# Tai-Wang/Depth-from-Motion

Hardware: AMD Instinct MI355X
Metric: cost-volumes/sec (higher is better)
Workload: dtype bf16; 1 GPU; nstar: plane-sweep cost-volume build B=8/GPU x (2C=512, D=112, 94x311), feats 256x94x311 bf16, fsf=4 csf=1; global_batch=8, parallelism=dp1, kernel=sweep_tile_kernel<LDS>, launch=lanes256_ppl8_planes2_chunk1_pipelined_cut64, autotuned=True, volume_layout=(B,2C,D,H,W) contiguous (the reference layout)

## Files before the change

### depth-from-motion_amd/csrc/plane_sweep.hip

```cpp
#include "plane_sweep_common.h"

#include <stdlib.h>
#include <string.h>

#include <algorithm>
#include <map>
#include <mutex>
#include <vector>

using namespace dfm;

namespace {

thread_local int g_last_kernel = 0;
#ifdef DFM_DEBUG_HOOKS
unsigned long long *g_trace = nullptr;
#endif

struct Launch {
    int kernel;
    int lanes;
    int lds_kib;
    int bpg;
    int planes;
    int band_chunk;
    int ppl;
    int align;
    int pair;
    int unpack;
    int pipe;
};

struct TuneKey {
    int v[9];
    bool operator<(const TuneKey &o) const { return memcmp(v, o.v, sizeof(v)) < 0; }
};
std::mutex g_tune_mu;
std::map<TuneKey, dfm_sweep_opts> g_tuned;

constexpr int PACK_PPL = 1;
__global__ void sweep_reset_kernel(int *flags, int n_flags, int *b, int *c)
{
    for (int i = threadIdx.x; i < n_flags; i += blockDim.x) flags[i] = 0;
    if (threadIdx.x == 0) { *b = 0; *c = 0; }
}

template <typename T>
__global__ __launch_bounds__(256) void pack_blocked_kernel(const T *__restrict__ src0,
                                                           const T *__restrict__ src1,
                                                           uint4 *__restrict__ dst0,
                                                           uint4 *__restrict__ dst1, int batch,
                                                           int C, int HW, int nblk, int *__restrict__ flags,
                                                           int W)
{
    constexpr int CB = elem<T>::CB;
    const int pix0 = blockIdx.x * (256 * PACK_PPL) + threadIdx.x;
    const int blk = blockIdx.y;
    const bool second = (int)blockIdx.z >= batch;
    const int b = second ? blockIdx.z - batch : blockIdx.z;
    const T *__restrict__ src = (second ? src1 : src0) + ((size_t)b * C + (size_t)blk * CB) * HW;
    uint4 *__restrict__ dst = (second ? dst1 : dst0) + ((size_t)b * nblk + blk) * HW;
    T v[PACK_PPL][CB];
#pragma unroll
    for (int i = 0; i < PACK_PPL; ++i) {
        const int pix = pix0 + i * 256;
#pragma unroll
        for (int j = 0; j < CB; ++j)
            v[i][j] = (blk * CB + j < C && pix < HW) ? src[(size_t)j * HW + pix] : T(0);
    }
#pragma unroll
    for (int i = 0; i < PACK_PPL; ++i) {
        const int pix = pix0 + i * 256;
        if (pix < HW) {
            uint4 q;
            memcpy(&q, v[i], 16);
            dst[pix] = q;
            if constexpr (sizeof(T) == 2) {
                bool odd_value = false;
                const uint32_t w4[4] = {q.x, q.y, q.z, q.w};
#pragma unroll
                for (int k = 0; k < 4; ++k)
#pragma unroll
                    for (int hbit = 0; hbit < 32; hbit += 16) {
                        const uint32_t e = (w4[k] >> hbit) & 0xffffu, ex = e & 0x7f80u;
                        odd_value |= ex == 0x7f80u || (ex == 0u && e != 0u);
                    }
                if (flags && odd_value) {
                    int *f = flags + (size_t)blockIdx.z * (HW / W) + pix / W;
                    if (__builtin_nontemporal_load(f) == 0) atomicOr(f, 1);
                }
            }
        }
    }
}

template <int CB>
__device__ __forceinline__ void blend(const Tap &t, const uint4 &qnw, const uint4 &qne,
                                      const uint4 &qsw, const uint4 &qse, float (&r)[CB])
{
    float a[CB], b[CB], c[CB], d[CB];
    unpack16(qnw, a);
    unpack16(qne, b);
    unpack16(qsw, c);
    unpack16(qse, d);
    const bool k0 = t.ok & 1u, k1 = t.ok & 2u, k2 = t.ok & 4u, k3 = t.ok & 8u;
#pragma unroll
    for (int j = 0; j < CB; ++j) {
        const float vnw = k0 ? a[j] : 0.0f;
        const float vne = k1 ? b[j] : 0.0f;
        const float vsw = k2 ? c[j] : 0.0f;
        const float vse = k3 ? d[j] : 0.0f;
        float acc = vnw * t.nw;
        acc = __builtin_fmaf(vne, t.ne, acc);
        acc = __builtin_fmaf(vsw, t.sw, acc);
        acc = __builtin_fmaf(vse, t.se, acc);
        r[j] = acc;
    }
}

template <int CB>
__device__ __forceinline__ void blend_nomask(const Tap &t, const uint4 &qnw, const uint4 &qne,
                                             const uint4 &qsw, const uint4 &qse, float (&r)[CB])
{
    float a[CB], b[CB], c[CB], d[CB];
    unpack16(qnw, a);
    unpack16(qne, b);
    unpack16(qsw, c);
    unpack16(qse, d);
#pragma unroll
    for (int j = 0; j < CB; ++j) {
        float acc = a[j] * t.nw;
        acc = __builtin_fmaf(b[j], t.ne, acc);
        acc = __builtin_fmaf(c[j], t.sw, acc);
        acc = __builtin_fmaf(d[j], t.se, acc);
        r[j] = acc;
    }
}

template <typename T>
__global__ __launch_bounds__(256) void sweep_gather_kernel(
    SweepGeom g, const uint4 *__restrict__ cur_blk, const uint4 *__restrict__ prev_blk,
    const float *__restrict__ depths, const float *__restrict__ P, const float *__restrict__ Pinv,
    const float *__restrict__ Tm, T *__restrict__ out)
{
    constexpr int CB = elem<T>::CB;
    const long long n = (long long)blockIdx.x * 256 + threadIdx.x;
    const int b = blockIdx.y;
    if (n >= g.N) return;
    const int hw = g.h_out * g.w_out;
    const int d = (int)(n / hw);
    const int rem = (int)(n - (long long)d * hw);
    const int hi = rem / g.w_out;
    const int wi = rem - hi * g.w_out;

    float cx, cy, px, py;
    sweep_point(g, P + b * 16, Pinv + b * 16, Tm + b * 16, depths[d], hi, wi, cx, cy, px, py,
                nullptr);
    const Tap tc = make_tap(cx, cy, g.h_in, g.w_in);
    const Tap tp = make_tap(px, py, g.h_in, g.w_in);

    const int HW = g.h_in * g.w_in;
    const int c00 = tc.iy * g.w_in + tc.ix, c01 = c00 + tc.dx;
    const int c10 = c00 + tc.dy * g.w_in, c11 = c10 + tc.dx;
    const int p00 = tp.iy * g.w_in + tp.ix, p01 = p00 + tp.dx;
    const int p10 = p00 + tp.dy * g.w_in, p11 = p10 + tp.dx;

    const uint4 *cb = cur_blk + (size_t)b * g.nblk * HW;
    const uint4 *pb = prev_blk + (size_t)b * g.nblk * HW;
    T *ocur = out + ((size_t)b * 2 * g.C) * g.N + n;
    T *oprev = ocur + (size_t)g.C * g.N;

    for (int blk = 0; blk < g.nblk; ++blk) {
        const uint4 qc0 = cb[c00], qc1 = cb[c01], qc2 = cb[c10], qc3 = cb[c11];
        const uint4 qp0 = pb[p00], qp1 = pb[p01], qp2 = pb[p10], qp3 = pb[p11];
// ... 4 lines not shown
#pragma unroll
        for (int j = 0; j < CB; ++j) {
            if (cbase + j < g.C) {
                ocur[(size_t)(cbase + j) * g.N] = elem<T>::store(rc[j]);
                oprev[(size_t)(cbase + j) * g.N] = elem<T>::store(rp[j]);
            }
        }
        cb += HW;
        pb += HW;
    }
}

template <typename T>
__global__ __launch_bounds__(256) void sweep_bwd_kernel(
    SweepGeom g, const T *__restrict__ gout, const float *__restrict__ depths,
    const float *__restrict__ P, const float *__restrict__ Pinv, const float *__restrict__ Tm,
    float *__restrict__ gcur, float *__restrict__ gprev)
{
    const long long n = (long long)blockIdx.x * 256 + threadIdx.x;
    const int b = blockIdx.y;
    if (n >= g.N) return;
    const int hw = g.h_out * g.w_out;
    const int d = (int)(n / hw);
    const int rem = (int)(n - (long long)d * hw);
    const int hi = rem / g.w_out;
    const int wi = rem - hi * g.w_out;
    float cx, cy, px, py;
    sweep_point(g, P + b * 16, Pinv + b * 16, Tm + b * 16, depths[d], hi, wi, cx, cy, px, py,
                nullptr);
    const Tap tc = make_tap(cx, cy, g.h_in, g.w_in);
    const Tap tp = make_tap(px, py, g.h_in, g.w_in);
    const int HW = g.h_in * g.w_in;
    const int c00 = tc.iy * g.w_in + tc.ix, c01 = c00 + tc.dx;
    const int c10 = c00 + tc.dy * g.w_in, c11 = c10 + tc.dx;
    const int p00 = tp.iy * g.w_in + tp.ix, p01 = p00 + tp.dx;
    const int p10 = p00 + tp.dy * g.w_in, p11 = p10 + tp.dx;
    const T *gc = gout + ((size_t)b * 2 * g.C) * g.N + n;
    const T *gp = gc + (size_t)g.C * g.N;
    float *dc = gcur + (size_t)b * g.C * HW;
    float *dp = gprev + (size_t)b * g.C * HW;
    for (int c = 0; c < g.C; ++c) {
        const float go_c = elem<T>::load(gc[(size_t)c * g.N]);
        const float go_p = elem<T>::load(gp[(size_t)c * g.N]);
        if (tc.ok & 1u) atomicAdd(dc + c00, go_c * tc.nw);
        if (tc.ok & 2u) atomicAdd(dc + c01, go_c * tc.ne);
        if (tc.ok & 4u) atomicAdd(dc + c10, go_c * tc.sw);
        if (tc.ok & 8u) atomicAdd(dc + c11, go_c * tc.se);
        if (tp.ok & 1u) atomicAdd(dp + p00, go_p * tp.nw);
        if (tp.ok & 2u) atomicAdd(dp + p01, go_p * tp.ne);
        if (tp.ok & 4u) atomicAdd(dp + p10, go_p * tp.sw);
        if (tp.ok & 8u) atomicAdd(dp + p11, go_p * tp.se);
        dc += HW;
        dp += HW;
    }
}

typedef uint32_t u32x4_t __attribute__((ext_vector_type(4)));

__device__ __forceinline__ void vol_store16(const u32x4_t &v, void *p)
{
    __builtin_nontemporal_store(v, (u32x4_t *)p);
}

__device__ __forceinline__ constexpr int waitcnt_vm(int n)
{
    return (n & 15) | (7 << 4) | (15 << 8) | ((n >> 4) << 14);
}

__device__ __forceinline__ int swz(int q) { return q ^ ((q >> 4) & 7); }

__device__ __forceinline__ uint32_t footprint(float x, float y, int H, int W, int &rN, int &rS,
                                              int &ix, float &fw, float &fn)
{
    const Tap t = make_tap(x, y, H, W);
    ix = (t.ok & 5u) ? t.ix : t.ix - ((t.ok & 10u) ? 1 : 0);
    rN = t.iy;
    rS = t.iy + t.dy;
    const bool fin = (fabsf(x) <= 3.0e38f) && (fabsf(y) <= 3.0e38f);
    fw = fin ? x - floorf(x) : 0.0f;
    fn = fin ? y - floorf(y) : 0.0f;
    return t.ok;
}

struct TileGrid {
    int batch;
    int bands;
    int band_pts;
    int planes;
    int dgroups;
    int blocks_per_group;
    int band_chunk;
    const int *flags;
    int mfma_unpack;
    int pair_stores;
    int align;
    unsigned long long *trace;
    int ablate;
};

constexpr int PIPE_BUF_SLOTS = 2504;
constexpr int PIPE_LDS_BYTES = (8 + 2 * PIPE_BUF_SLOTS) * 16;
template <int N> struct IntC { static constexpr int value = N; };

template <typename T, int NT, bool LDS, int V, bool PIPE = false, bool MXK = false>
__device__ __forceinline__ int tile_body(
    const int bid, const SweepGeom &g, const SweepFast &fast, const TileGrid &tg, int lds_slots,
    const uint4 *__restrict__ cur_blk, const uint4 *__restrict__ prev_blk,
    const float *__restrict__ depths, const float *__restrict__ P,
    const float *__restrict__ Pinv, const float *__restrict__ Tm, T *__restrict__ out,
    int *__restrict__ spill_list, int blk_lo_ovr = -1, int blk_hi_ovr = -1, bool retry_inline = false)
{
    constexpr int CB = elem<T>::CB;
    static_assert(V == 4 || V == 8, "points per lane");
    static_assert(V * sizeof(T) == 16 || V * sizeof(T) == 8, "8- or 16-byte stores");
    static_assert(LDS || !PIPE, "the pipelined body is an LDS-staged body");
    static_assert(!MXK || (LDS && sizeof(T) == 2 && V == 8), "matrix-core unpack: bf16, LDS taps, 8 points per lane");
    constexpr int VW = V * (int)sizeof(T) / 4;
    constexpr int PAD = 8;
    constexpr int SLAB = 8;
    extern __shared__ __attribute__((aligned(16))) uint4 lds[];
    int *bb = (int *)lds;

    const int tid = threadIdx.x;
    const int batch = tg.batch;
    const int b = bid % batch;
    int th = bid / batch;
    const int band_in = th % tg.band_chunk;
    th /= tg.band_chunk;
    const int dgroup = th % tg.dgroups;
    th /= tg.dgroups;
    const int half = th & 1;
    th >>= 1;
    const int nchunks = (tg.bands + tg.band_chunk - 1) / tg.band_chunk;
    const int band = (th % nchunks) * tg.band_chunk + band_in;
    const int group = th / nchunks;
    if (band >= tg.bands) return 0;
    const int blk_lo = blk_lo_ovr >= 0 ? blk_lo_ovr : group * tg.blocks_per_group;
    const int blk_hi = blk_lo_ovr >= 0 ? min(blk_hi_ovr, g.nblk) : min(blk_lo + tg.blocks_per_group, g.nblk);
    const int lanes_per_plane = NT / tg.planes;
    const int d_tile = dgroup * tg.planes + tid / lanes_per_plane;
    const int tid_p = tid % lanes_per_plane;
    const long long hw_ll = (long long)g.h_out * g.w_out;
    const long long a0 = (d_tile * hw_ll) & ~7ll;
    const long long a1 = d_tile >= g.D - 1 ? g.N : (((d_tile + 1) * hw_ll) & ~7ll);
    const long long base = a0 & ~(long long)(tg.align - 1);
    const long long t_end = d_tile < g.D ? min(base + (long long)(band + 1) * tg.band_pts, a1) : 0;
    const long long n0 = base + (long long)band * tg.band_pts + (long long)tid_p * V;
    const bool active = n0 >= a0 && n0 < t_end;
    const int W = g.w_in, H = g.h_in;
    const int HW = H * W;

    if (LDS) {
        if (tid == 0) {
            bb[0] = 0x7fffffff;
            bb[1] = -1;
            lds[SLAB] = make_uint4(0u, 0u, 0u, 0u);
            if constexpr (PIPE) lds[SLAB + PIPE_BUF_SLOTS] = make_uint4(0u, 0u, 0u, 0u);
        }
        __syncthreads();
    }

    int qN[V], qS[V];
    float fw[V], fn[V];
    uint32_t okbits = 0;
    int ymin = 0x7fffffff, ymax = -1;
    if (active) {
        const int hw = g.h_out * g.w_out;
        int d = (int)(n0 / hw);
        int rem = (int)(n0 - (long long)d * hw);
        int hi = rem / g.w_out;
        int wi = rem - hi * g.w_out;
        const float *Pb = P + b * 16, *Pib = Pinv + b * 16, *Tb = Tm + b * 16;
#pragma unroll
        for (int j = 0; j < V; ++j) {
            float sx, sy;
            if (half) sweep_point_map<1>(g, fast, Pb, Pib, Tb, depths[d], hi, wi, sx, sy);
            else sweep_point_map<0>(g, fast, Pb, Pib, Tb, depths[d], hi, wi, sx, sy);
            int rN, rS, ix;
            uint32_t ok = footprint(sx, sy, H, W, rN, rS, ix, fw[j], fn[j]);
            if (LDS && d != d_tile) ok = 0;
            qN[j] = rN * W + ix;
            qS[j] = rS * W + ix;
            okbits |= ok << (4 * j);
            if (ok) { ymin = min(ymin, rN); ymax = max(ymax, rS); }
            if (++wi == g.w_out) { wi = 0; if (++hi == g.h_out) { hi = 0; ++d; } }
            __builtin_amdgcn_sched_barrier(0);
        }
    }
    T *o = out + ((size_t)b * 2 * g.C + (size_t)half * g.C) * g.N + n0;
    const uint32_t full = (V == 8) ? 0xffffffffu : 0xffffu;
    typedef uint32_t u32x2_t __attribute__((ext_vector_type(2)));
    const bool all_in = __all(!active || okbits == full);

    int cnt = 0, nslots = 0;
    int ta[V][4];
    const uint4 *src = (half ? prev_blk : cur_blk) + ((size_t)b * g.nblk + blk_lo) * HW;
    if (LDS) {
#pragma unroll
        for (int s = 32; s > 0; s >>= 1) {
            ymin = min(ymin, __shfl_xor(ymin, s));
            ymax = max(ymax, __shfl_xor(ymax, s));
        }
        if ((tid & 63) == 0) { atomicMin(&bb[0], ymin); atomicMax(&bb[1], ymax); }
        __syncthreads();
        const int y0 = bb[0], y1 = bb[1];
        if (y1 < y0) {
            if (active) {
                for (int c = blk_lo * CB; c < min(blk_hi * CB, g.C); ++c) {
                    if constexpr (VW == 4) {
                        const u32x4_t z = {0u, 0u, 0u, 0u};
                        __builtin_nontemporal_store(z, (u32x4_t *)(o + (size_t)c * g.N));
                    } else {
                        const u32x2_t z = {0u, 0u};
                        __builtin_nontemporal_store(z, (u32x2_t *)(o + (size_t)c * g.N));
                    }
                }
            }
            return 0;
        }
        cnt = (y1 - y0 + 1) * W;
        nslots = (PAD + cnt + 1 + 7) & ~7;
        const bool fits = PIPE ? nslots <= min(PIPE_BUF_SLOTS, (lds_slots - SLAB) / 2)
                               : SLAB + nslots <= lds_slots;
        if (!fits) {
            if (retry_inline) return 1;
            if (tid == 0 && blk_lo_ovr <= 0) spill_list[1 + atomicAdd(&spill_list[0], 1)] = bid;
            return 0;
        }
        if constexpr (MXK) {
            const int nrows = y1 - y0 + 1;
            const int *rf = tg.flags + ((size_t)half * batch + b) * H + y0;
            bool odd_row = false;
            for (int r = tid & 63; r < nrows; r += 64) odd_row |= rf[r] != 0;
            if (__any(odd_row)) {
                if (retry_inline) return 2;
                if (tid == 0 && blk_lo_ovr <= 0) spill_list[1 + atomicAdd(&spill_list[0], 1)] = bid;
                return 0;
            }
        }
        const int off = PAD - y0 * W;
        constexpr int ZERO = SLAB << 4;
#pragma unroll
        for (int j = 0; j < V; ++j) {
            const uint32_t ok = (okbits >> (4 * j)) & 15u;
            const int a = qN[j] + off, c = qS[j] + off;
            ta[j][0] = (ok & 1u) ? (SLAB + swz(a)) << 4 : ZERO;
            ta[j][1] = (ok & 2u) ? (SLAB + swz(a + 1)) << 4 : ZERO;
            ta[j][2] = (ok & 4u) ? (SLAB + swz(c)) << 4 : ZERO;
            ta[j][3] = (ok & 8u) ? (SLAB + swz(c + 1)) << 4 : ZERO;
        }
        src += (size_t)y0 * W;
    } else {
        if (!active) return 0;
#pragma unroll
        for (int j = 0; j < V; ++j) {
            const bool any = (okbits >> (4 * j)) & 15u;
            qN[j] = any ? qN[j] : 0;
            qS[j] = any ? qS[j] : 0;
        }
    }
    const int wave = tid >> 6, lane = tid & 63;
    typedef __bf16 mxs_bf16x4 __attribute__((ext_vector_type(4)));
    mxs_bf16x4 mx_sel;
    if constexpr (MXK) {
        const int i = lane & 3;
        const uint32_t s2[2] = {i == 0 ? 0x3f80u : i == 1 ? 0x3f800000u : 0u,
                                i == 2 ? 0x3f80u : i == 3 ? 0x3f800000u : 0u};
        __builtin_memcpy(&mx_sel, s2, 8);
    }
#ifdef DFM_DEBUG_HOOKS
    unsigned long long *tr = (LDS && tg.trace && (bid % 509) == 0 && tid == 0)
                                 ? tg.trace + (size_t)(bid / 509) * 64 : nullptr;
    int tri = 0;
#endif
#ifndef DFM_DEBUG_HOOKS
#define TRACE_STAMP() do {} while (0)
#define ABLATE(bit) false
#else
#define ABLATE(bit) ((tg.ablate & (bit)) != 0)
#define TRACE_STAMP()                                                                       \
    do {                                                                                    \
        if (tr && tri < 64) {                                                               \
            unsigned long long t_;                                                          \
            asm volatile("s_memtime %0\n\ts_waitcnt lgkmcnt(0)" : "=s"(t_)::"memory");       \
            tr[tri++] = t_;                                                                 \
        }                                                                                   \
    } while (0)
#endif
    TRACE_STAMP();

    auto compute_block = [&](int blk, const uint4 *gsrc, auto bufc, auto mxc, uint32_t (&pk)[CB][VW]) {
        constexpr int BOFF = decltype(bufc)::value * PIPE_BUF_SLOTS * 16;
        constexpr bool MX = decltype(mxc)::value != 0 && MXK;
        static_assert(BOFF < 65536, "ds_read_b128 immediate offset");
        if (ABLATE(4)) {
#pragma unroll
            for (int k = 0; k < CB; ++k)
#pragma unroll
                for (int j = 0; j < VW; ++j) pk[k][j] = (uint32_t)qN[j] + k + blk;
        } else if constexpr (MX) {
            typedef __bf16 mx_bf16x4 __attribute__((ext_vector_type(4)));
            typedef float mx_f32x4 __attribute__((ext_vector_type(4)));
#define DFM_TAP_READ(dst, addr) \
    asm volatile("ds_read_b128 %0, %1 offset:%2" : "=v"(dst) : "v"(addr), "i"(BOFF))
            const mx_f32x4 z4 = {0.0f, 0.0f, 0.0f, 0.0f};
            auto cvt_half = [&](uint32_t lo, uint32_t hi, float *f) {
                mx_bf16x4 bfrag;
                const uint32_t h[2] = {lo, hi};
                __builtin_memcpy(&bfrag, h, 8);
                const mx_f32x4 d4 = __builtin_amdgcn_mfma_f32_4x4x4bf16_1k(mx_sel, bfrag, z4, 0, 0, 0);
                f[0] = d4[0]; f[1] = d4[1]; f[2] = d4[2]; f[3] = d4[3];
            };
            u32x4_t q[2][4];
            float keep[CB];
#pragma unroll
            for (int c4 = 0; c4 < 4; ++c4) DFM_TAP_READ(q[0][c4], ta[0][c4]);
// ... 151 lines not shown
        }
#pragma unroll
        for (int k = 0; k < CB; ++k) {
            if (cbase + k < g.C && (!ABLATE(2) || pk[k][0] == 0x12345u)) {
                if constexpr (VW == 4) {
                    u32x4_t v = {pk[k][0], pk[k][1], pk[k][2], pk[k][3]};
                    vol_store16(v, o + (size_t)(cbase + k) * g.N);
                } else {
                    u32x2_t v = {pk[k][0], pk[k][1]};
                    __builtin_nontemporal_store(v, (u32x2_t *)(o + (size_t)(cbase + k) * g.N));
                }
            }
        }
    };
    auto compute_store = [&](int blk, const uint4 *gsrc, auto bufc, auto mxc) {
        uint32_t pk[CB][VW];
        compute_block(blk, gsrc, bufc, mxc, pk);
        store_block(blk, pk);
    };

    if constexpr (!LDS) {
        for (int blk = blk_lo; blk < blk_hi; ++blk) {
            compute_store(blk, src, IntC<0>{}, IntC<0>{});
            src += HW;
        }
    } else {
        auto stage = [&](int buf_slot0, const uint4 *gsrc) {
            if (ABLATE(1)) return;
            for (int s0 = wave * 64; s0 < nslots; s0 += NT) {
                const int p = swz(s0 + lane) - PAD;
                if (p >= 0 && p < cnt)
                    __builtin_amdgcn_global_load_lds(
                        (const __attribute__((address_space(1))) void *)(gsrc + p),
                        (__attribute__((address_space(3))) void *)(lds + buf_slot0 + s0), 16, 0, 0);
            }
        };
        if constexpr (!PIPE) {
            for (int blk = blk_lo; blk < blk_hi; ++blk) {
                stage(SLAB, src);
                TRACE_STAMP();
                __syncthreads();
                TRACE_STAMP();
                if (active) compute_store(blk, src, IntC<0>{}, IntC<MXK ? 1 : 0>{});
                TRACE_STAMP();
                src += HW;
                __syncthreads();
                TRACE_STAMP();
            }
        } else {
            const bool wave_stores = __any(active) != 0;
            const bool paired = VW == 2 && tg.pair_stores;
            auto wait_rows = [&]() {
                if (wave_stores && !ABLATE(2) && !paired)
                    asm volatile("s_waitcnt vmcnt(%0)\n\ts_barrier" ::"i"(CB) : "memory");
                else if (wave_stores && !ABLATE(2))
                    asm volatile("s_waitcnt vmcnt(%0)\n\ts_barrier" ::"i"(CB / 2) : "memory");
                else
                    asm volatile("s_waitcnt vmcnt(0)\n\ts_barrier" ::: "memory");
            };
            stage(SLAB, src);
            TRACE_STAMP();
            asm volatile("s_waitcnt vmcnt(0) lgkmcnt(0)\n\ts_barrier" ::: "memory");
            for (int blk = blk_lo;;) {
                if (blk + 1 < blk_hi) stage(SLAB + PIPE_BUF_SLOTS, src + HW);
                TRACE_STAMP();
                if (active) compute_store(blk, src, IntC<0>{}, IntC<MXK ? 1 : 0>{});
                TRACE_STAMP();
                src += HW;
                if (++blk >= blk_hi) break;
                wait_rows();
                TRACE_STAMP();
                if (blk + 1 < blk_hi) stage(SLAB, src + HW);
                TRACE_STAMP();
                if (active) compute_store(blk, src, IntC<1>{}, IntC<MXK ? 1 : 0>{});
                TRACE_STAMP();
                src += HW;
                if (++blk >= blk_hi) break;
                wait_rows();
                TRACE_STAMP();
            }
        }
    }
#undef DFM_TAP_READ
    return 0;
}

#ifndef DFM_TILE_WAVES
#define DFM_TILE_WAVES 1
#endif
template <typename T, int NT, bool LDS, int V, bool PIPE = false, bool MXK = false>
__global__ __launch_bounds__(NT, (LDS ? (V * sizeof(T) == 8 ? 4 : (MXK ? 2 : DFM_TILE_WAVES)) : 1)) void sweep_tile_kernel(
    SweepGeom g, SweepFast fast, TileGrid tg, int lds_slots, const uint4 *__restrict__ cur_blk,
    const uint4 *__restrict__ prev_blk, const float *__restrict__ depths,
    const float *__restrict__ P, const float *__restrict__ Pinv, const float *__restrict__ Tm,
    T *__restrict__ out, int *__restrict__ spill_list)
{
    int st = tile_body<T, NT, LDS, V, PIPE, MXK>(blockIdx.x, g, fast, tg, lds_slots, cur_blk, prev_blk, depths, P,
                                                 Pinv, Tm, out, spill_list, -1, -1, PIPE);
    if constexpr (PIPE) {
        if constexpr (MXK) {
            if (st == 2) {
                __syncthreads();
                st = tile_body<T, NT, true, V, true, false>(blockIdx.x, g, fast, tg, lds_slots, cur_blk, prev_blk,
                                                            depths, P, Pinv, Tm, out, spill_list, -1, -1, true);
            }
        }
        if (st == 1) {
            __syncthreads();
            constexpr bool INPLACE3 = V * sizeof(T) == 16;
            st = tile_body<T, NT, true, V, false, false>(blockIdx.x, g, fast, tg, lds_slots, cur_blk, prev_blk, depths,
                                                         P, Pinv, Tm, out, spill_list, -1, -1, INPLACE3);
            if constexpr (INPLACE3) {
                if (st == 1) {
                    __syncthreads();
                    tile_body<T, NT, false, V>(blockIdx.x, g, fast, tg, 0, cur_blk, prev_blk, depths, P, Pinv, Tm,
                                               out, nullptr);
                }
            }
        }
    }
}

template <typename T, int NT, int V>
__global__ __launch_bounds__(NT) void sweep_spill_kernel(
    SweepGeom g, SweepFast fast, TileGrid tg, const uint4 *__restrict__ cur_blk,
    const uint4 *__restrict__ prev_blk, const float *__restrict__ depths,
    const float *__restrict__ P, const float *__restrict__ Pinv, const float *__restrict__ Tm,
    T *__restrict__ out, int *__restrict__ spill_list)
{
    const int count = spill_list[0];
    for (int i = blockIdx.x; i < count; i += gridDim.x)
        tile_body<T, NT, false, V>(spill_list[1 + i], g, fast, tg, 0, cur_blk, prev_blk, depths, P,
                                   Pinv, Tm, out, nullptr);
}

template <typename T, int NT, int V>
__global__ __launch_bounds__(NT, (V * sizeof(T) == 8 ? 4 : DFM_TILE_WAVES)) void sweep_respill_kernel(
    SweepGeom g, SweepFast fast, TileGrid tg, int lds_slots, int groups, int blocks_per_group,
    const uint4 *__restrict__ cur_blk, const uint4 *__restrict__ prev_blk,
    const float *__restrict__ depths, const float *__restrict__ P, const float *__restrict__ Pinv,
    const float *__restrict__ Tm, T *__restrict__ out, const int *__restrict__ list_in,
    int *__restrict__ list_out)
{
    const int count = list_in[0];
    for (int i = blockIdx.x; i < count * groups; i += gridDim.x) {
        const int grp = i % groups;
        tile_body<T, NT, true, V>(list_in[1 + i / groups], g, fast, tg, lds_slots, cur_blk, prev_blk,
                                  depths, P, Pinv, Tm, out, list_out, grp * blocks_per_group,
                                  (grp + 1) * blocks_per_group);
        __syncthreads();
    }
}

template <typename T>
__global__ __launch_bounds__(256) void sweep_patch_kernel(
    SweepGeom g, SweepFast fast, int align, const uint4 *__restrict__ cur_blk,
    const uint4 *__restrict__ prev_blk, const float *__restrict__ depths,
    const float *__restrict__ P, const float *__restrict__ Pinv, const float *__restrict__ Tm,
    T *__restrict__ out)
{
    constexpr int CB = elem<T>::CB;
    const int d_next = blockIdx.x + 1;
    const int half = blockIdx.y, b = blockIdx.z;
    const long long hw = (long long)g.h_out * g.w_out;
    const long long edge = d_next * hw;
    const int d = d_next - 1;
    const int HW = g.h_in * g.w_in;
    const uint4 *mb = (half ? prev_blk : cur_blk) + (size_t)b * g.nblk * HW;
    (void)align;
    for (long long n = (edge & ~7ll) + (threadIdx.x >> 5); n < edge; n += 8) {
        const int rem = (int)(n - (long long)d * hw);
        const int hi = rem / g.w_out, wi = rem - hi * g.w_out;
        float sx, sy;
        if (half) sweep_point_map<1>(g, fast, P + b * 16, Pinv + b * 16, Tm + b * 16, depths[d], hi, wi, sx, sy);
        else sweep_point_map<0>(g, fast, P + b * 16, Pinv + b * 16, Tm + b * 16, depths[d], hi, wi, sx, sy);
        const Tap t = make_tap(sx, sy, g.h_in, g.w_in);
        const int i00 = t.iy * g.w_in + t.ix, i01 = i00 + t.dx;
        const int i10 = i00 + t.dy * g.w_in, i11 = i10 + t.dx;
        T *o = out + ((size_t)b * 2 * g.C + (size_t)half * g.C) * g.N + n;
        for (int blk = threadIdx.x & 31; blk < g.nblk; blk += 32) {
            const uint4 *q = mb + (size_t)blk * HW;
            float r[CB];
            blend<CB>(t, q[i00], q[i01], q[i10], q[i11], r);
#pragma unroll
            for (int k = 0; k < CB; ++k)
                if (blk * CB + k < g.C) o[(size_t)(blk * CB + k) * g.N] = elem<T>::store(r[k]);
        }
    }
}

__global__ __launch_bounds__(256) void sweep_grid_kernel(SweepGeom g, int b,
                                                         const float *__restrict__ depths,
                                                         const float *__restrict__ P,
                                                         const float *__restrict__ Pinv,
                                                         const float *__restrict__ Tm,
                                                         float *__restrict__ cur_grid,
                                                         float *__restrict__ prev_grid)
{
    const long long n = (long long)blockIdx.x * 256 + threadIdx.x;
    if (n >= g.N) return;
    const int hw = g.h_out * g.w_out;
    const int d = (int)(n / hw);
    const int rem = (int)(n - (long long)d * hw);
    const int hi = rem / g.w_out;
    const int wi = rem - hi * g.w_out;
    float cx, cy, px, py, norm[4];
    sweep_point(g, P + b * 16, Pinv + b * 16, Tm + b * 16, depths[d], hi, wi, cx, cy, px, py, norm);
    cur_grid[2 * n] = norm[0];
    cur_grid[2 * n + 1] = norm[1];
    prev_grid[2 * n] = norm[2];
    prev_grid[2 * n + 1] = norm[3];
}

__global__ void camera_prepare_kernel(const float *__restrict__ cam2img, int rows, int cols,
                                      int batch, float *__restrict__ P, float *__restrict__ Pinv)
{
    const int b = blockIdx.x * blockDim.x + threadIdx.x;
    if (b >= batch) return;
    float m[4][8];
    const float *src = cam2img + (size_t)b * rows * cols;
    const int use_rows = rows == 4 ? 3 : rows;
#pragma unroll
    for (int i = 0; i < 4; ++i)
#pragma unroll
        for (int j = 0; j < 4; ++j) {
            float v = i == j ? 1.0f : 0.0f;
            if (i < use_rows && j < cols) v = src[i * cols + j];
            m[i][j] = v;
            m[i][j + 4] = i == j ? 1.0f : 0.0f;
            P[b * 16 + i * 4 + j] = v;
        }
#pragma unroll
    for (int c = 0; c < 4; ++c) {
        int piv = c;
        float best = fabsf(m[c][c]);
#pragma unroll
        for (int r = 0; r < 4; ++r)
            if (r > c && fabsf(m[r][c]) > best) { best = fabsf(m[r][c]); piv = r; }
#pragma unroll
        for (int r = 0; r < 4; ++r)
            if (r == piv && r != c) {
#pragma unroll
                for (int j = 0; j < 8; ++j) { const float t = m[c][j]; m[c][j] = m[r][j]; m[r][j] = t; }
            }
        const float inv = 1.0f / m[c][c];
#pragma unroll
        for (int j = 0; j < 8; ++j) m[c][j] *= inv;
#pragma unroll
        for (int r = 0; r < 4; ++r)
            if (r != c) {
                const float f = m[r][c];
#pragma unroll
                for (int j = 0; j < 8; ++j) m[r][j] = m[r][j] - f * m[c][j];
            }
    }
#pragma unroll
    for (int i = 0; i < 4; ++i)
#pragma unroll
        for (int j = 0; j < 4; ++j) Pinv[b * 16 + i * 4 + j] = m[i][j + 4];
}

int check_desc(const dfm_sweep_desc *d)
{
    if (!d) return set_error(DFM_ERR_INVALID_ARG, "desc is NULL");
    if (d->batch <= 0 || d->channels <= 0 || d->h_in <= 0 || d->w_in <= 0 || d->num_depths <= 0 ||
        d->h_out <= 0 || d->w_out <= 0)
        return set_error(DFM_ERR_INVALID_ARG, "non-positive size in dfm_sweep_desc");
    if (d->dtype != DFM_F32 && d->dtype != DFM_BF16)
        return set_error(DFM_ERR_UNSUPPORTED, "dtype must be DFM_F32 or DFM_BF16");
    if ((long long)d->h_in * d->w_in >= (1ll << 31) / 64)
        return set_error(DFM_ERR_UNSUPPORTED, "feature map too large for 32-bit tap offsets");
    if (d->batch > 32767) return set_error(DFM_ERR_UNSUPPORTED, "batch > 32767");
    return DFM_OK;
}

SweepGeom make_geom(const dfm_sweep_desc *d)
{
    SweepGeom g;
    g.C = d->channels;
    g.h_in = d->h_in;
    g.w_in = d->w_in;
    g.D = d->num_depths;
    g.h_out = d->h_out;
    g.w_out = d->w_out;
    const int CB = d->dtype == DFM_BF16 ? 8 : 4;
    g.nblk = (d->channels + CB - 1) / CB;
    g.flip = d->flip;
    g.fsf = d->feat_sample_factor;
    g.csf = d->cost_sample_factor;
    g.scale = d->img_scale_factor;
    g.crop_x = d->crop_x;
    g.crop_y = d->crop_y;
    g.org_w = d->org_w;
    g.N = (long long)d->num_depths * d->h_out * d->w_out;
    return g;
}

size_t blocked_bytes(const dfm_sweep_desc *d)
{
    const int CB = d->dtype == DFM_BF16 ? 8 : 4;
    const size_t nblk = (d->channels + CB - 1) / CB;
    size_t one = (size_t)d->batch * nblk * d->h_in * d->w_in * 16;
    return (one + 255) & ~(size_t)255;
}

size_t row_flag_bytes(const dfm_sweep_desc *d)
{
    return (((size_t)2 * d->batch * d->h_in * 4) + 255) & ~(size_t)255;
}

size_t flag_bytes(const dfm_sweep_desc *d)
{
    const int V = d->dtype == DFM_BF16 ? 8 : 4;
    const long long hw = (long long)d->h_out * d->w_out;
    const long long bands = (hw + 7 + 63 + 64ll * V - 1) / (64ll * V);
    const long long nblk = (d->channels + V - 1) / V;
    return ((size_t)(1 + bands * d->num_depths * 2 * d->batch * nblk) * 4 + 255) & ~(size_t)255;
}

SweepFast make_fast(const dfm_sweep_desc *d)
{
    SweepFast fast;
    fast.scale_is_one = d->img_scale_factor == 1.0f;
    int e = 0;
    const float m = frexpf(d->feat_sample_factor, &e);
    fast.fsf_pow2 = (m == 0.5f) && e > -60 && e < 60;
    fast.inv_fsf = 1.0f / d->feat_sample_factor;
    return fast;
}

int resolve(const dfm_sweep_desc *d, const dfm_sweep_opts *o, Launch &L)
{
    const int CB = d->dtype == DFM_BF16 ? 8 : 4;
    L.kernel = o ? o->kernel : 0;
    L.lanes = o && o->lanes_per_workgroup ? o->lanes_per_workgroup : 256;
    L.lds_kib = o && o->lds_kib ? o->lds_kib : 0;
    L.bpg = o && o->blocks_per_group ? o->blocks_per_group : (1 << 20);
    L.planes = o && o->planes_per_workgroup ? o->planes_per_workgroup : 2;
    L.band_chunk = o && o->bands_per_chunk ? o->bands_per_chunk : 1;
    L.ppl = o && o->points_per_lane ? o->points_per_lane : CB;
    L.align = o && o->store_align_points ? o->store_align_points : 64;
    if (L.align != 8 && L.align != 16 && L.align != 32 && L.align != 64)
        return set_error(DFM_ERR_INVALID_ARG, "opts: store_align_points in {8,16,32,64}");
    L.pair = o && o->pair_stores ? (o->pair_stores == 1) : 1;
    if (o && (o->unpack < 0 || o->unpack > 2)) return set_error(DFM_ERR_INVALID_ARG, "opts: unpack must be 0, 1 or 2");
    L.unpack = o && o->unpack ? (o->unpack == 1) : 1;
    L.pipe = o && o->pipeline ? o->pipeline : 2;
    if (L.pipe != 1 && L.pipe != 2) return set_error(DFM_ERR_INVALID_ARG, "opts: pipeline must be 0, 1 or 2");
    if (!L.lds_kib) L.lds_kib = L.pipe >= 2 ? 80 : 52;
    if (L.kernel < 0 || L.kernel > 5) return set_error(DFM_ERR_INVALID_ARG, "opts: kernel must be 0..5");
    if (L.lanes != 128 && L.lanes != 256 && L.lanes != 512 && L.lanes != 1024)
        return set_error(DFM_ERR_INVALID_ARG, "opts: lanes_per_workgroup in {128,256,512,1024}");
    if (L.lds_kib < 4 || L.lds_kib > 160 || L.bpg < 1 || L.planes < 1 || L.band_chunk < 1)
        return set_error(DFM_ERR_INVALID_ARG, "opts: 4 <= lds_kib <= 160, blocks_per_group / planes / bands_per_chunk >= 1");
    if (L.ppl != CB && !(L.ppl == 4 && CB == 8 && L.lanes >= 256))
        return set_error(DFM_ERR_INVALID_ARG, "opts: points_per_lane is 16/sizeof(T), or 4 for bf16 with >= 256 lanes");
    if (L.lanes == 1024 && L.ppl != 4)
        return set_error(DFM_ERR_INVALID_ARG, "opts: 1024 lanes need points_per_lane = 4");
    return DFM_OK;
}

template <typename T, int NT, int V>
int launch_tiles(int which, const dfm_sweep_desc *d, const SweepGeom &g, const Launch &L,
                 const uint4 *cur_blk, const uint4 *prev_blk, const float *depths, const float *P,
                 const float *Pinv, const float *Tm, T *out, int *spill_list, hipStream_t st)
{
    const int lds_bytes = L.lds_kib * 1024;
    const int bpg = which == 2 ? std::min(L.bpg, g.nblk) : g.nblk;
    const int groups = (g.nblk + bpg - 1) / bpg;
    const long long hw = (long long)g.h_out * g.w_out;
    TileGrid tg;
    tg.batch = d->batch;
    tg.planes = std::max(1, std::min(L.planes, NT / 64));
    while ((NT / 64) % tg.planes) --tg.planes;
    tg.dgroups = (g.D + tg.planes - 1) / tg.planes;
    const long long per_plane = (long long)(NT / tg.planes) * V;
    tg.align = (int)std::min<long long>(L.align, per_plane & -per_plane);
    const long long am = tg.align - 1;
    tg.bands = (int)((hw + 7 + am + per_plane - 1) / per_plane);
    tg.band_pts = (int)((((hw + 7 + am + tg.bands - 1) / tg.bands) + am) & ~am);
    tg.blocks_per_group = bpg;
    tg.band_chunk = std::max(1, std::min(L.band_chunk, tg.bands));
    tg.trace = nullptr;
    tg.ablate = 0;
    tg.pair_stores = L.pair;
    tg.mfma_unpack = L.unpack;
    tg.flags = (const int *)((const char *)spill_list + 2 * flag_bytes(d));
#ifdef DFM_DEBUG_HOOKS
    tg.trace = g_trace;
    {
        const char *ab = getenv("DFM_ABLATE");
        tg.ablate = ab ? atoi(ab) : 0;
    }
#endif
    const long long nchunks = (tg.bands + tg.band_chunk - 1) / tg.band_chunk;
    const long long nb = nchunks * tg.band_chunk * tg.dgroups * 2 * d->batch * groups;
    if (nb > 2147483647ll) return set_error(DFM_ERR_UNSUPPORTED, "too many lattice points");
    if ((size_t)(nb + 1) * 4 > flag_bytes(d)) return set_error(DFM_ERR_WORKSPACE, "spill list too small");
    int rc = DFM_OK;
    const SweepFast fast = make_fast(d);
    if (which == 2) {
        int *spill2 = (int *)((char *)spill_list + flag_bytes(d));
        constexpr bool CAN_MX = sizeof(T) == 2 && V == 8;
        if (L.pipe >= 2 && CAN_MX && L.unpack) {
            if constexpr (CAN_MX) {
                const void *kern = (const void *)sweep_tile_kernel<T, NT, true, V, true, true>;
                rc = ensure_dynamic_lds(kern, PIPE_LDS_BYTES);
                if (rc != DFM_OK) return rc;
                hipLaunchKernelGGL((sweep_tile_kernel<T, NT, true, V, true, true>), dim3((unsigned)nb), dim3(NT),
                                   PIPE_LDS_BYTES, st, g, fast, tg, std::min(lds_bytes, PIPE_LDS_BYTES) / 16,
                                   cur_blk, prev_blk, depths, P, Pinv, Tm, out, spill_list);
            }
        } else if (L.pipe >= 2) {
            const void *kern = (const void *)sweep_tile_kernel<T, NT, true, V, true>;
            rc = ensure_dynamic_lds(kern, PIPE_LDS_BYTES);
            if (rc != DFM_OK) return rc;
            hipLaunchKernelGGL((sweep_tile_kernel<T, NT, true, V, true>), dim3((unsigned)nb), dim3(NT),
                               PIPE_LDS_BYTES, st, g, fast, tg, std::min(lds_bytes, PIPE_LDS_BYTES) / 16,
                               cur_blk, prev_blk, depths, P, Pinv, Tm, out, spill_list);
        } else {
            const void *kern = (const void *)sweep_tile_kernel<T, NT, true, V>;
            rc = ensure_dynamic_lds(kern, lds_bytes);
            if (rc != DFM_OK) return rc;
            hipLaunchKernelGGL((sweep_tile_kernel<T, NT, true, V>), dim3((unsigned)nb), dim3(NT),
                               lds_bytes, st, g, fast, tg, lds_bytes / 16, cur_blk, prev_blk, depths, P,
                               Pinv, Tm, out, spill_list);
        }
        const bool queues = !(L.pipe >= 2 && V * sizeof(T) == 16);
        if (queues) {
            const int BIG = L.lds_kib < 16 ? lds_bytes : 144 * 1024;
            const void *rk = (const void *)sweep_respill_kernel<T, NT, V>;
            rc = ensure_dynamic_lds(rk, BIG);
            if (rc != DFM_OK) return rc;
            const int rgroups = std::min(8, g.nblk);
            const int rbpg = (g.nblk + rgroups - 1) / rgroups;
            hipLaunchKernelGGL((sweep_respill_kernel<T, NT, V>), dim3(1024), dim3(NT), BIG, st, g, fast,
                               tg, BIG / 16, rgroups, rbpg, cur_blk, prev_blk, depths, P, Pinv, Tm, out,
                               (const int *)spill_list, spill2);
        }
        if (queues)
            hipLaunchKernelGGL((sweep_spill_kernel<T, NT, V>), dim3(512), dim3(NT), 16, st, g, fast, tg,
                               cur_blk, prev_blk, depths, P, Pinv, Tm, out, spill2);
        if (g.D > 1 && hw % 8 != 0)
            hipLaunchKernelGGL(sweep_patch_kernel<T>, dim3(g.D - 1, 2, d->batch), dim3(256), 0, st,
                               g, fast, tg.align, cur_blk, prev_blk, depths, P, Pinv, Tm, out);
    } else {
        hipLaunchKernelGGL((sweep_tile_kernel<T, NT, false, V>), dim3((unsigned)nb), dim3(NT), 16,
                           st, g, fast, tg, 0, cur_blk, prev_blk, depths, P, Pinv, Tm, out,
                           (int *)nullptr);
    }
    return DFM_OK;
}

template <typename T>
int launch_fwd(const dfm_sweep_desc *d, const Launch &L, const void *cur, const void *prev,
               const float *depths, const float *P, const float *Pinv, const float *Tm, void *out,
               void *ws, hipStream_t st)
{
    const SweepGeom g = make_geom(d);
    const int HW = d->h_in * d->w_in;
    if ((L.kernel == 4 || L.kernel == 5 || (L.kernel == 0 && d->cost_sample_factor >= 1.5f)) &&
        sweep_clt_supported(d, out)) {
        return sweep_clt_launch(d, cur, prev, depths, P, Pinv, Tm, out, ws, (void *)st, false, L.kernel != 4);
    }
    uint4 *cur_blk = (uint4 *)ws;
    uint4 *prev_blk = (uint4 *)((char *)ws + blocked_bytes(d));
    dim3 pg((HW + 256 * PACK_PPL - 1) / (256 * PACK_PPL), g.nblk, 2 * d->batch);
    int *feat_flags = (int *)((char *)ws + 2 * blocked_bytes(d) + 2 * flag_bytes(d));
    const bool timed = profile_mark(st, false);
    hipLaunchKernelGGL(sweep_reset_kernel, dim3(1), dim3(256), 0, st, feat_flags, 2 * d->batch * d->h_in,
                       (int *)((char *)ws + 2 * blocked_bytes(d)),
                       (int *)((char *)ws + 2 * blocked_bytes(d) + flag_bytes(d)));
    hipLaunchKernelGGL(pack_blocked_kernel<T>, pg, dim3(256), 0, st, (const T *)cur, (const T *)prev,
                       cur_blk, prev_blk, d->batch, g.C, HW, g.nblk, feat_flags, d->w_in);
    constexpr int CB = elem<T>::CB;
    const bool vec_ok = g.N % CB == 0 && ((uintptr_t)out & 15) == 0;
    int which = !vec_ok ? 1 : (d->cost_sample_factor < 1.5f ? 2 : 3);
    if (L.kernel == 1 || (L.kernel == 3 && vec_ok)) which = L.kernel;
    if (L.kernel == 2 && vec_ok) which = 2;
    int rc = DFM_OK;
    if (which == 1) {
        const long long nb = (g.N + 255) / 256;
        if (nb > 2147483647ll) return set_error(DFM_ERR_UNSUPPORTED, "too many lattice points");
        dim3 grid((unsigned)nb, d->batch);
        hipLaunchKernelGGL(sweep_gather_kernel<T>, grid, dim3(256), 0, st, g, cur_blk, prev_blk,
                           depths, P, Pinv, Tm, (T *)out);
    } else {
        int *spill_list = (int *)((char *)ws + 2 * blocked_bytes(d));
#define DFM_TILES(NT, V)                                                                            \
    rc = launch_tiles<T, NT, V>(which, d, g, L, cur_blk, prev_blk, depths, P, Pinv, Tm, (T *)out,   \
                                spill_list, st)
        if (L.ppl == CB) {
            if (L.lanes == 128) DFM_TILES(128, CB);
            else if (L.lanes == 256) DFM_TILES(256, CB);
            else if (L.lanes == 512) DFM_TILES(512, CB);
            else if constexpr (CB == 4) DFM_TILES(1024, 4);
        } else {
            if constexpr (CB == 8) {
                if (L.lanes == 256) DFM_TILES(256, 4);
                else if (L.lanes == 512) DFM_TILES(512, 4);
                else DFM_TILES(1024, 4);
            }
        }
#undef DFM_TILES
    }
    if (timed) profile_mark(st, true);
    if (rc != DFM_OK) return rc;
    g_last_kernel = which;
    HIP_TRY(hipGetLastError());
    return DFM_OK;
}

int run_fwd(const dfm_sweep_desc *desc, const Launch &L, const void *cur, const void *prev,
            const float *depths, const float *cam2img, const float *cam2img_inv,
            const float *cur2prev, void *out, void *workspace, hipStream_t st)
{
    if (desc->dtype == DFM_F32)
        return launch_fwd<float>(desc, L, cur, prev, depths, cam2img, cam2img_inv, cur2prev, out,
                                 workspace, st);
    return launch_fwd<bf16_t>(desc, L, cur, prev, depths, cam2img, cam2img_inv, cur2prev, out,
                              workspace, st);
}

size_t fwd_workspace_bytes(const dfm_sweep_desc *desc)
{
    return std::max(2 * blocked_bytes(desc) + 2 * flag_bytes(desc) + row_flag_bytes(desc),
                    sweep_clt_workspace_bytes(desc));
}

int check_fwd_args(const dfm_sweep_desc *desc, const void *cur, const void *prev,
                   const float *depths, const float *cam2img, const float *cam2img_inv,
                   const float *cur2prev, void *out, void *workspace, size_t workspace_bytes)
{
    int rc = check_desc(desc);
    if (rc != DFM_OK) return rc;
    if (!cur || !prev || !depths || !cam2img || !cam2img_inv || !cur2prev || !out)
        return set_error(DFM_ERR_INVALID_ARG, "NULL device pointer");
    if (!workspace || workspace_bytes < fwd_workspace_bytes(desc))
        return set_error(DFM_ERR_WORKSPACE, "workspace smaller than dfm_plane_sweep_workspace_bytes");
    if (((uintptr_t)workspace & 15) || ((uintptr_t)out & 1))
        return set_error(DFM_ERR_INVALID_ARG, "workspace must be 16-byte aligned");
    return DFM_OK;
}

int tune_key(const dfm_sweep_desc *d, TuneKey &k)
{
    int dev = 0;
    HIP_TRY(hipGetDevice(&dev));
    const int v[9] = {dev, d->batch, d->channels, d->h_in, d->w_in, d->num_depths, d->h_out,
                      d->w_out, d->dtype};
    memcpy(k.v, v, sizeof(v));
    return DFM_OK;
}

bool takes_lds_tiles(const dfm_sweep_desc *d, const void *out)
{
    const int CB = d->dtype == DFM_BF16 ? 8 : 4;
// ... 229 lines not shown
```

Baseline: 1478 cost-volumes/s.

## Fold reset into pack kernel and patch depth-boundary points inline in tile kernel

Removes the separate reset kernel: the pack kernel now zeroes the spill counters and writes a per-block odd-value flag using a block-wide OR instead of atomics on per-row flags. Flags become per (channel block, 256-pixel run), so the tile kernel checks only the channel blocks it touches. When the pipelined path runs without spill queues, the depth-boundary patch work runs inside the tile kernel (first band, first wavefront) rather than in a separate patch kernel launch. This cuts kernel launches and atomics, but adds serial boundary work and a wait on outstanding memory operations inside the main kernel, and the flag buffer grows.

```diff
diff --git a/depth-from-motion_amd/csrc/plane_sweep.hip b/depth-from-motion_amd/csrc/plane_sweep.hip
--- a/depth-from-motion_amd/csrc/plane_sweep.hip
+++ b/depth-from-motion_amd/csrc/plane_sweep.hip
@@ -38,58 +38,50 @@
 std::mutex g_tune_mu;
 std::map<TuneKey, dfm_sweep_opts> g_tuned;
 
-constexpr int PACK_PPL = 1;
-__global__ void sweep_reset_kernel(int *flags, int n_flags, int *b, int *c)
-{
-    for (int i = threadIdx.x; i < n_flags; i += blockDim.x) flags[i] = 0;
-    if (threadIdx.x == 0) { *b = 0; *c = 0; }
-}
+constexpr int PACK_NT = 256;
 
 template <typename T>
-__global__ __launch_bounds__(256) void pack_blocked_kernel(const T *__restrict__ src0,
-                                                           const T *__restrict__ src1,
-                                                           uint4 *__restrict__ dst0,
-                                                           uint4 *__restrict__ dst1, int batch,
-                                                           int C, int HW, int nblk, int *__restrict__ flags,
-                                                           int W)
+__global__ __launch_bounds__(PACK_NT) void pack_blocked_kernel(const T *__restrict__ src0,
+                                                               const T *__restrict__ src1,
+                                                               uint4 *__restrict__ dst0,
+                                                               uint4 *__restrict__ dst1, int batch,
+                                                               int C, int HW, int nblk, int *__restrict__ flags,
+                                                               int *__restrict__ spill_a,
+                                                               int *__restrict__ spill_b)
 {
     constexpr int CB = elem<T>::CB;
-    const int pix0 = blockIdx.x * (256 * PACK_PPL) + threadIdx.x;
+    const int pix = blockIdx.x * PACK_NT + threadIdx.x;
     const int blk = blockIdx.y;
     const bool second = (int)blockIdx.z >= batch;
     const int b = second ? blockIdx.z - batch : blockIdx.z;
     const T *__restrict__ src = (second ? src1 : src0) + ((size_t)b * C + (size_t)blk * CB) * HW;
     uint4 *__restrict__ dst = (second ? dst1 : dst0) + ((size_t)b * nblk + blk) * HW;
-    T v[PACK_PPL][CB];
-#pragma unroll
-    for (int i = 0; i < PACK_PPL; ++i) {
-        const int pix = pix0 + i * 256;
-#pragma unroll
-        for (int j = 0; j < CB; ++j)
-            v[i][j] = (blk * CB + j < C && pix < HW) ? src[(size_t)j * HW + pix] : T(0);
-    }
-#pragma unroll
-    for (int i = 0; i < PACK_PPL; ++i) {
-        const int pix = pix0 + i * 256;
-        if (pix < HW) {
-            uint4 q;
-            memcpy(&q, v[i], 16);
-            dst[pix] = q;
-            if constexpr (sizeof(T) == 2) {
-                bool odd_value = false;
-                const uint32_t w4[4] = {q.x, q.y, q.z, q.w};
-#pragma unroll
-                for (int k = 0; k < 4; ++k)
-#pragma unroll
-                    for (int hbit = 0; hbit < 32; hbit += 16) {
-                        const uint32_t e = (w4[k] >> hbit) & 0xffffu, ex = e & 0x7f80u;
-                        odd_value |= ex == 0x7f80u || (ex == 0u && e != 0u);
-                    }
-                if (flags && odd_value) {
-                    int *f = flags + (size_t)blockIdx.z * (HW / W) + pix / W;
-                    if (__builtin_nontemporal_load(f) == 0) atomicOr(f, 1);
+    if (blockIdx.x == 0 && blockIdx.y == 0 && blockIdx.z == 0 && threadIdx.x == 0) { *spill_a = 0; *spill_b = 0; }
+    T v[CB];
+#pragma unroll
+    for (int j = 0; j < CB; ++j)
+        v[j] = (blk * CB + j < C && pix < HW) ? src[(size_t)j * HW + pix] : T(0);
+    bool odd_value = false;
+    if (pix < HW) {
+        uint4 q;
+        memcpy(&q, v, 16);
+        dst[pix] = q;
+        if constexpr (sizeof(T) == 2) {
+            const uint32_t w4[4] = {q.x, q.y, q.z, q.w};
+#pragma unroll
+            for (int k = 0; k < 4; ++k)
+#pragma unroll
+                for (int hbit = 0; hbit < 32; hbit += 16) {
+                    const uint32_t e = (w4[k] >> hbit) & 0xffffu, ex = e & 0x7f80u;
+                    odd_value |= ex == 0x7f80u || (ex == 0u && e != 0u);
                 }
-            }
+        }
+    }
+    if constexpr (sizeof(T) == 2) {
+        if (flags) {
+            const int any_odd = __syncthreads_or(odd_value);
+            if (threadIdx.x == 0)
+                flags[((size_t)blockIdx.z * nblk + blk) * gridDim.x + blockIdx.x] = any_odd ? 1 : 0;
         }
     }
 }
@@ -260,6 +252,37 @@
     return t.ok;
 }
 
+template <typename T>
+__device__ __forceinline__ void patch_point(const SweepGeom &g, const SweepFast &fast, int half, int b, int d,
+                                            long long n, int blk0, int blk_end,
+                                            const uint4 *__restrict__ cur_blk, const uint4 *__restrict__ prev_blk,
+                                            const float *__restrict__ depths, const float *__restrict__ P,
+                                            const float *__restrict__ Pinv, const float *__restrict__ Tm,
+                                            T *__restrict__ out)
+{
+    constexpr int CB = elem<T>::CB;
+    const long long hw = (long long)g.h_out * g.w_out;
+    const int HW = g.h_in * g.w_in;
+    const uint4 *mb = (half ? prev_blk : cur_blk) + (size_t)b * g.nblk * HW;
+    const int rem = (int)(n - (long long)d * hw);
+    const int hi = rem / g.w_out, wi = rem - hi * g.w_out;
+    float sx, sy;
+    if (half) sweep_point_map<1>(g, fast, P + b * 16, Pinv + b * 16, Tm + b * 16, depths[d], hi, wi, sx, sy);
+    else sweep_point_map<0>(g, fast, P + b * 16, Pinv + b * 16, Tm + b * 16, depths[d], hi, wi, sx, sy);
+    const Tap t = make_tap(sx, sy, g.h_in, g.w_in);
+    const int i00 = t.iy * g.w_in + t.ix, i01 = i00 + t.dx;
+    const int i10 = i00 + t.dy * g.w_in, i11 = i10 + t.dx;
+    T *o = out + ((size_t)b * 2 * g.C + (size_t)half * g.C) * g.N + n;
+    for (int blk = blk0; blk < blk_end; blk += 32) {
+        const uint4 *q = mb + (size_t)blk * HW;
+        float r[CB];
+        blend<CB>(t, q[i00], q[i01], q[i10], q[i11], r);
+#pragma unroll
+        for (int k = 0; k < CB; ++k)
+            if (blk * CB + k < g.C) o[(size_t)(blk * CB + k) * g.N] = elem<T>::store(r[k]);
+    }
+}
+
 struct TileGrid {
     int batch;
     int bands;
@@ -269,6 +292,7 @@
     int blocks_per_group;
     int band_chunk;
     const int *flags;
+    int patch_inline;
     int mfma_unpack;
     int pair_stores;
     int align;
@@ -370,6 +394,18 @@
     typedef uint32_t u32x2_t __attribute__((ext_vector_type(2)));
     const bool all_in = __all(!active || okbits == full);
 
+    auto patch_boundary = [&]() {
+        if constexpr (LDS) {
+            const long long edge = d_tile * hw_ll;
+            if (!tg.patch_inline || band != 0 || tid_p >= 64 || d_tile < 1 || d_tile >= g.D || (edge & 7) == 0)
+                return;
+            asm volatile("s_waitcnt vmcnt(0)" ::: "memory");
+            for (long long n = (edge & ~7ll) + ((tid & 63) >> 5); n < edge; n += 2)
+                patch_point<T>(g, fast, half, b, d_tile - 1, n, blk_lo + (tid & 31), blk_hi, cur_blk, prev_blk,
+                               depths, P, Pinv, Tm, out);
+        }
+    };
+
     int cnt = 0, nslots = 0;
     int ta[V][4];
     const uint4 *src = (half ? prev_blk : cur_blk) + ((size_t)b * g.nblk + blk_lo) * HW;
@@ -394,6 +430,7 @@
                     }
                 }
             }
+            patch_boundary();
             return 0;
         }
         cnt = (y1 - y0 + 1) * W;
@@ -406,10 +443,14 @@
             return 0;
         }
         if constexpr (MXK) {
-            const int nrows = y1 - y0 + 1;
-            const int *rf = tg.flags + ((size_t)half * batch + b) * H + y0;
+            const int nruns = (HW + PACK_NT - 1) / PACK_NT;
+            const int run0 = y0 * W / PACK_NT, nrun = ((y1 + 1) * W - 1) / PACK_NT - run0 + 1;
+            const int *rf = tg.flags + (((size_t)half * batch + b) * g.nblk + blk_lo) * nruns + run0;
             bool odd_row = false;
-            for (int r = tid & 63; r < nrows; r += 64) odd_row |= rf[r] != 0;
+            for (int i = tid & 63; i < nrun * (blk_hi - blk_lo); i += 64) {
+                const int k = i / nrun;
+                odd_row |= rf[(size_t)k * nruns + (i - k * nrun)] != 0;
+            }
             if (__any(odd_row)) {
                 if (retry_inline) return 2;
                 if (tid == 0 && blk_lo_ovr <= 0) spill_list[1 + atomicAdd(&spill_list[0], 1)] = bid;
@@ -727,6 +768,7 @@
         }
     }
 #undef DFM_TAP_READ
+    patch_boundary();
     return 0;
 }
 
@@ -804,34 +846,13 @@
     const float *__restrict__ P, const float *__restrict__ Pinv, const float *__restrict__ Tm,
     T *__restrict__ out)
 {
-    constexpr int CB = elem<T>::CB;
     const int d_next = blockIdx.x + 1;
     const int half = blockIdx.y, b = blockIdx.z;
-    const long long hw = (long long)g.h_out * g.w_out;
-    const long long edge = d_next * hw;
-    const int d = d_next - 1;
-    const int HW = g.h_in * g.w_in;
-    const uint4 *mb = (half ? prev_blk : cur_blk) + (size_t)b * g.nblk * HW;
+    const long long edge = d_next * (long long)g.h_out * g.w_out;
     (void)align;
-    for (long long n = (edge & ~7ll) + (threadIdx.x >> 5); n < edge; n += 8) {
-        const int rem = (int)(n - (long long)d * hw);
-        const int hi = rem / g.w_out, wi = rem - hi * g.w_out;
-        float sx, sy;
-        if (half) sweep_point_map<1>(g, fast, P + b * 16, Pinv + b * 16, Tm + b * 16, depths[d], hi, wi, sx, sy);
-        else sweep_point_map<0>(g, fast, P + b * 16, Pinv + b * 16, Tm + b * 16, depths[d], hi, wi, sx, sy);
-        const Tap t = make_tap(sx, sy, g.h_in, g.w_in);
-        const int i00 = t.iy * g.w_in + t.ix, i01 = i00 + t.dx;
-        const int i10 = i00 + t.dy * g.w_in, i11 = i10 + t.dx;
-        T *o = out + ((size_t)b * 2 * g.C + (size_t)half * g.C) * g.N + n;
-        for (int blk = threadIdx.x & 31; blk < g.nblk; blk += 32) {
-            const uint4 *q = mb + (size_t)blk * HW;
-            float r[CB];
-            blend<CB>(t, q[i00], q[i01], q[i10], q[i11], r);
-#pragma unroll
-            for (int k = 0; k < CB; ++k)
-                if (blk * CB + k < g.C) o[(size_t)(blk * CB + k) * g.N] = elem<T>::store(r[k]);
-        }
-    }
+    for (long long n = (edge & ~7ll) + (threadIdx.x >> 5); n < edge; n += 8)
+        patch_point<T>(g, fast, half, b, d_next - 1, n, threadIdx.x & 31, g.nblk, cur_blk, prev_blk, depths, P,
+                       Pinv, Tm, out);
 }
 
 __global__ __launch_bounds__(256) void sweep_grid_kernel(SweepGeom g, int b,
@@ -951,7 +972,10 @@
 
 size_t row_flag_bytes(const dfm_sweep_desc *d)
 {
-    return (((size_t)2 * d->batch * d->h_in * 4) + 255) & ~(size_t)255;
+    const int CB = d->dtype == DFM_BF16 ? 8 : 4;
+    const size_t nblk = (d->channels + CB - 1) / CB;
+    const size_t nruns = ((size_t)d->h_in * d->w_in + PACK_NT - 1) / PACK_NT;
+    return (((size_t)2 * d->batch * nblk * nruns * 4) + 255) & ~(size_t)255;
 }
 
 size_t flag_bytes(const dfm_sweep_desc *d)
@@ -1030,6 +1054,7 @@
     tg.ablate = 0;
     tg.pair_stores = L.pair;
     tg.mfma_unpack = L.unpack;
+    tg.patch_inline = 0;
     tg.flags = (const int *)((const char *)spill_list + 2 * flag_bytes(d));
 #ifdef DFM_DEBUG_HOOKS
     tg.trace = g_trace;
@@ -1047,6 +1072,8 @@
     if (which == 2) {
         int *spill2 = (int *)((char *)spill_list + flag_bytes(d));
         constexpr bool CAN_MX = sizeof(T) == 2 && V == 8;
+        const bool queues = !(L.pipe >= 2 && V * sizeof(T) == 16);
+        tg.patch_inline = !queues;
         if (L.pipe >= 2 && CAN_MX && L.unpack) {
             if constexpr (CAN_MX) {
                 const void *kern = (const void *)sweep_tile_kernel<T, NT, true, V, true, true>;
@@ -1071,7 +1098,6 @@
                                lds_bytes, st, g, fast, tg, lds_bytes / 16, cur_blk, prev_blk, depths, P,
                                Pinv, Tm, out, spill_list);
         }
-        const bool queues = !(L.pipe >= 2 && V * sizeof(T) == 16);
         if (queues) {
             const int BIG = L.lds_kib < 16 ? lds_bytes : 144 * 1024;
             const void *rk = (const void *)sweep_respill_kernel<T, NT, V>;
@@ -1086,7 +1112,7 @@
         if (queues)
             hipLaunchKernelGGL((sweep_spill_kernel<T, NT, V>), dim3(512), dim3(NT), 16, st, g, fast, tg,
                                cur_blk, prev_blk, depths, P, Pinv, Tm, out, spill2);
-        if (g.D > 1 && hw % 8 != 0)
+        if (queues && g.D > 1 && hw % 8 != 0)
             hipLaunchKernelGGL(sweep_patch_kernel<T>, dim3(g.D - 1, 2, d->batch), dim3(256), 0, st,
                                g, fast, tg.align, cur_blk, prev_blk, depths, P, Pinv, Tm, out);
     } else {
@@ -1103,21 +1129,20 @@
                void *ws, hipStream_t st)
 {
     const SweepGeom g = make_geom(d);
-    const int HW = d->h_in * d->w_in;
     if ((L.kernel == 4 || L.kernel == 5 || (L.kernel == 0 && d->cost_sample_factor >= 1.5f)) &&
         sweep_clt_supported(d, out)) {
         return sweep_clt_launch(d, cur, prev, depths, P, Pinv, Tm, out, ws, (void *)st, false, L.kernel != 4);
     }
     uint4 *cur_blk = (uint4 *)ws;
     uint4 *prev_blk = (uint4 *)((char *)ws + blocked_bytes(d));
-    dim3 pg((HW + 256 * PACK_PPL - 1) / (256 * PACK_PPL), g.nblk, 2 * d->batch);
+    const int HW = d->h_in * d->w_in;
+    dim3 pg((HW + PACK_NT - 1) / PACK_NT, g.nblk, 2 * d->batch);
     int *feat_flags = (int *)((char *)ws + 2 * blocked_bytes(d) + 2 * flag_bytes(d));
     const bool timed = profile_mark(st, false);
-    hipLaunchKernelGGL(sweep_reset_kernel, dim3(1), dim3(256), 0, st, feat_flags, 2 * d->batch * d->h_in,
+    hipLaunchKernelGGL(pack_blocked_kernel<T>, pg, dim3(PACK_NT), 0, st, (const T *)cur, (const T *)prev,
+                       cur_blk, prev_blk, d->batch, g.C, HW, g.nblk, feat_flags,
                        (int *)((char *)ws + 2 * blocked_bytes(d)),
                        (int *)((char *)ws + 2 * blocked_bytes(d) + flag_bytes(d)));
-    hipLaunchKernelGGL(pack_blocked_kernel<T>, pg, dim3(256), 0, st, (const T *)cur, (const T *)prev,
-                       cur_blk, prev_blk, d->batch, g.C, HW, g.nblk, feat_flags, d->w_in);
     constexpr int CB = elem<T>::CB;
     const bool vec_ok = g.N % CB == 0 && ((uintptr_t)out & 15) == 0;
     int which = !vec_ok ? 1 : (d->cost_sample_factor < 1.5f ? 2 : 3);
```

New measurement: 1478 cost-volumes/s (median of 2 runs). No clear change (+0.0%).
